# kamperh/segmentalist

Measured on AMD Instinct MI355X. Metric: Gibbs sweeps/sec (10k utts, D=100, K=1000) at 1/2/4/8 MI355X, higher is better.
Workload: dtype fp16 one-product filter + fp16x2 second stage, float32 reference arithmetic for the results; 1 GPU; SegmentalKMeansWordseg batch-synchronous sweep (BASELINE.json configs[2]); utterances=10000, landmarks_per_utt=20, n_slices_max=6, embeddings=1050000, D=100, K=1000, parallelism=utterance shards x1, ONE all-gather of the packed block statistics per sweep, collective=none (single process), sweep_launch=plain launches, corpus=one device holds all rows, device_memory_allocated_bytes_rank0=1237140480, components_after=815

## Files before the change

segmentalist_amd/csrc/segk_segment.hip:

```cpp
#include "segk_kmeans_dev.h"
#include "segk_segment_dev.h"


__global__ void k_kmeans_segment(segk_corpus c, segk_kmeans m, const int32_t *utts, int utt0, int n_utts,
                                 int n_min, int n_max, double wip, segk_cand cand, uint8_t *boundaries,
                                 int32_t *old_tok, int32_t *new_tok, int32_t *new_k, int32_t *n_old,
                                 int32_t *n_new, int32_t *n_flag, double *out_total, int32_t *status, int band_cap,
                                 int wave_bytes)
{
    extern __shared__ __attribute__((aligned(16))) char smem[];
    (void)n_min;
    const int lane = threadIdx.x & 63, wv = threadIdx.x >> 6;
    const int slot = blockIdx.x * (blockDim.x >> 6) + wv;
    if (slot >= n_utts) return;
    const int u = utts ? utts[slot] : utt0 + slot;
    const int N = c.lengths[u];
    const int W = (n_max > 0 && n_max < N) ? n_max : N;
    const int nb = N * W;
    const int64_t triMax = (int64_t)c.N_max * (c.N_max + 1) / 2;
    const int32_t *vid = c.vec_ids + (int64_t)u * triMax;
    const double *dur = c.durations + (int64_t)u * triMax;
    const bool band = c.band_ids != nullptr && c.band_W == W && W > 0;
    const int32_t *bandi = band ? c.band_ids + (int64_t)u * c.N_max * c.band_W : nullptr;
    const double *bandd = band ? c.band_dur + (int64_t)u * c.N_max * c.band_W : nullptr;
    uint8_t *gbnd = boundaries + (int64_t)u * c.N_max;

    char *base = smem + (size_t)wv * wave_bytes;
    double *bvec = (double *)base;
    double *gam = bvec + band_cap;
    int32_t *bk = (int32_t *)(gam + c.N_max + 1);
    int32_t *bid = bk + band_cap;
    int32_t *l_old = bid + band_cap;
    int32_t *l_new = l_old + c.N_max;
    int32_t *l_newk = l_new + c.N_max;
    int32_t *l_cnt = l_newk + c.N_max;
    uint8_t *l_bnd = (uint8_t *)(l_cnt + 2);

    for (int i = lane; i < nb; i += 64) {
        const int t = i / W + 1, w = i % W, s = t - 1 - w;
        int id = -1;
        double v = NEG_INF_D;
        int k = -1;
        if (s >= 0) {
            const int j = t * (t - 1) / 2 + s;
            id = band ? bandi[i] : vid[j];
            if (id >= 0) {
                k = cand.k[id];
                const double dd = band ? bandd[i] : dur[j];
                v = isnan(dd) ? NEG_INF_D : cand.s[id] * dd;
            }
        }
        bid[i] = id;
        bk[i] = k;
        bvec[i] = v + wip;
    }
    for (int j = lane; j < N; j += 64) l_bnd[j] = gbnd[j];
    WAVE_SYNC();
    if (lane == 0) {
#define V_(t, s) bvec[((t) - 1) * W + ((t) - 1 - (s))]
#define ID_(t, s) (((t) - 1 - (s)) < W ? bid[((t) - 1) * W + ((t) - 1 - (s))] : vid[(t) * ((t) - 1) / 2 + (s)])
        int no = 0, jp = 0;
        for (int j = 0; j < N; j++)
            if (l_bnd[j]) {
                int id = ID_(j + 1, jp);
                if (id >= 0) l_old[no++] = id;
                jp = j + 1;
            }
        gam[0] = 0.0;
        for (int t = 1; t < N; t++) {
            int lo = t - W < 0 ? 0 : t - W;
            double best = NEG_INF_D;
            for (int s = lo; s < t; s++) {
                double v = V_(t, s) + gam[s];
                if (v > best) best = v;
            }
            gam[t] = best;
        }
        for (int j = 0; j < N; j++) l_bnd[j] = 0;
        l_bnd[N - 1] = 1;
        int t = N;
        double total = 0.0;
        int lo = 0;
        for (;;) {
            lo = t - W < 0 ? 0 : t - W;
            bool all_inf = true;
            for (int s = lo; s < t; s++)
                if (V_(t, s) + gam[s] != NEG_INF_D) { all_inf = false; break; }
            if (all_inf) {
                while (all_inf) {
                    t = t - 1;
                    if (t == 0) break;
                    lo = t - W < 0 ? 0 : t - W;
                    all_inf = true;
                    for (int s = lo; s < t; s++)
                        if (V_(t, s) + gam[s] != NEG_INF_D) { all_inf = false; break; }
                }
                l_bnd[(t - 1 + N) % N] = 1;
            }
            int k = 1;
            if (t > 0) {
                double best = NEG_INF_D;
                bool first = true;
                for (int s = t - 1; s >= lo; s--) {
                    double v = V_(t, s) + gam[s];
                    if (first || v > best) { best = v; k = t - s; first = false; }
                }
                total += V_(t, t - k);
            } else {
                total += V_(N, N - 1);
            }
            if (t - k - 1 < 0) break;
            l_bnd[t - k - 1] = 1;
            t = t - k;
        }
        int nn = 0, bad = 0, nf = 0;
        const int Kact = *m.K;
        jp = 0;
        for (int j = 0; j < N; j++)
            if (l_bnd[j]) {
                int tt = j + 1, w = tt - 1 - jp;
                if (w >= W || bid[(tt - 1) * W + w] < 0) bad = 1;
                else {
                    l_new[nn] = bid[(tt - 1) * W + w];
                    l_newk[nn] = bk[(tt - 1) * W + w];
                    if (l_newk[nn] >= Kact) nf++;
                    nn++;
                }
                jp = j + 1;
            }
        out_total[u] = total;
        n_old[u] = no;
        n_new[u] = nn;
        if (n_flag) n_flag[u] = nf;
        l_cnt[0] = no;
        l_cnt[1] = nn;
        if (bad) atomicOr(status, 1);
#undef V_
#undef ID_
    }
    WAVE_SYNC();
    const int no = l_cnt[0], nn = l_cnt[1];
    for (int j = lane; j < N; j += 64) gbnd[j] = l_bnd[j];
    for (int j = lane; j < no; j += 64) old_tok[(int64_t)u * c.N_max + j] = l_old[j];
    for (int j = lane; j < c.N_max; j += 64) {
        if (j < nn) new_tok[(int64_t)u * c.N_max + j] = l_new[j];
        new_k[(int64_t)u * c.N_max + j] = j < nn ? l_newk[j] : -1;
    }
}

__global__ __launch_bounds__(256) void k_kmeans_segment_w8(segk_corpus c, segk_kmeans m, const int32_t *utts, int utt0, int n_utts,
                                    int n_max, double wip, segk_cand cand, uint8_t *boundaries, int32_t *old_tok,
                                    int32_t *new_tok, int32_t *new_k, int32_t *n_old, int32_t *n_new, int32_t *n_flag,
                                    double *out_total, int32_t *status, int band_cap, int wave_bytes)
{
    extern __shared__ __attribute__((aligned(16))) char smem[];
    const int lane = threadIdx.x & 63, wv = threadIdx.x >> 6;
    const int slot = blockIdx.x * (blockDim.x >> 6) + wv;
    SEGK_TSTAMP(0, 0);
    if (slot >= n_utts) return;
    const int u = utts ? utts[slot] : utt0 + slot;
    const int N = c.lengths[u];
    const int W = (n_max > 0 && n_max < N) ? n_max : N;
    const int64_t triMax = (int64_t)c.N_max * (c.N_max + 1) / 2;
    const int32_t *vid = c.vec_ids + (int64_t)u * triMax;
    const double *dur = c.durations + (int64_t)u * triMax;
    const bool band = c.band_ids != nullptr && c.band_W == W && W > 0;
    const int32_t *bandi = band ? c.band_ids + (int64_t)u * c.N_max * c.band_W : nullptr;
    const double *bandd = band ? c.band_dur + (int64_t)u * c.N_max * c.band_W : nullptr;
    uint8_t *gbnd = boundaries + (int64_t)u * c.N_max;

    char *base = smem + (size_t)wv * wave_bytes;
    double *bvec = (double *)base;
    double *gam = bvec + c.N_max * 8;
    int32_t *bk = (int32_t *)(gam + c.N_max + 12);
    int32_t *bid = bk + band_cap;
    int32_t *l_old = bid + band_cap;
    int32_t *l_new = l_old + c.N_max;
    int32_t *l_newk = l_new + c.N_max;
    int32_t *l_cnt = l_newk + c.N_max;

    {
        const int w = lane & 7;
        for (int z0 = 0; z0 < N; z0 += 32) {
            int id[4], kq[4];
            double dd[4], sc[4];
#pragma unroll
            for (int z = 0; z < 4; z++) {
                const int r = z0 + 8 * z + (lane >> 3), t = r + 1, sp = t - 1 - w;
                id[z] = -1;
                dd[z] = 0.0;
                if (r < N && w < W && sp >= 0) {
                    const int j = t * (t - 1) / 2 + sp;
                    id[z] = band ? bandi[r * W + w] : vid[j];
                    dd[z] = band ? bandd[r * W + w] : dur[j];
                }
            }
#pragma unroll
            for (int z = 0; z < 4; z++) {
                kq[z] = -1;
                sc[z] = 0.0;
                if (id[z] >= 0) {
                    kq[z] = cand.k[id[z]];
                    sc[z] = cand.s[id[z]];
                }
            }
#pragma unroll
            for (int z = 0; z < 4; z++) {
                const int r = z0 + 8 * z + (lane >> 3);
                if (r < N) {
                    double v = NEG_INF_D;
                    if (id[z] >= 0) v = isnan(dd[z]) ? NEG_INF_D : sc[z] * dd[z];
                    if (w < W) {
                        bid[r * W + w] = id[z];
                        bk[r * W + w] = kq[z];
                    }
                    bvec[r * 8 + w] = v + wip;
                }
            }
        }
    }
    const unsigned long long oldb = __ballot(lane < N && gbnd[lane < N ? lane : 0] != 0);
    WAVE_SYNC();
    SEGK_TSTAMP(0, 1);
    {
        const int no_ = seg_old_tokens_wave(bid, vid, N, W, oldb, l_old, lane);
        if (lane == 0) l_cnt[0] = no_;
    }
    double total;
    {
        unsigned long long newb_, keep_;
        int e_, k_, x_, f_;
        seg_w8_uniform(bvec, gam, bid, bk, N, W, *m.K, l_new, l_newk, l_cnt, &total, lane, newb_, keep_, e_, k_, x_, f_);
    }
    WAVE_SYNC();
    SEGK_TSTAMP(0, 2);
    if (lane == 0) {
        out_total[u] = total;
        n_old[u] = l_cnt[0];
        n_new[u] = l_cnt[1];
        if (n_flag) n_flag[u] = l_cnt[4];
        if (l_cnt[5]) atomicOr(status, 1);
    }
    WAVE_SYNC();
    const int no = l_cnt[0], nn = l_cnt[1];
    const unsigned long long newb = ((unsigned long long)(unsigned int)l_cnt[3] << 32) | (unsigned int)l_cnt[2];
    if (lane < N) gbnd[lane] = (uint8_t)((newb >> lane) & 1ull);
    for (int j = lane; j < no; j += 64) old_tok[(int64_t)u * c.N_max + j] = l_old[j];
    for (int j = lane; j < c.N_max; j += 64) {
        if (j < nn) new_tok[(int64_t)u * c.N_max + j] = l_new[j];
        new_k[(int64_t)u * c.N_max + j] = j < nn ? l_newk[j] : -1;
    }
    SEGK_TSTAMP_MAX(0, 3);
}

__device__ double dev_logsumexp(const double *a, int n)
{
    double mx = a[0], s = 0.0;
    for (int j = 1; j < n; j++)
        if (a[j] > mx) mx = a[j];
    for (int j = 0; j < n; j++) s += exp(a[j] - mx);
    return log(s) + mx;
}

__global__ void k_dp_tri(int kind, const double *vecs, const int32_t *Ns, const int64_t *offs, int n_prob,
                         int n_min, int n_max, double log_p_continue, double anneal_temp,
                         const double *uniforms, int64_t u_stride, uint8_t *bounds, int64_t b_stride,
                         double *totals, int32_t *n_draws, int32_t *status, double *work, int64_t w_stride)
{
    const int p = blockIdx.x * blockDim.x + threadIdx.x;
    if (p >= n_prob) return;
    const int N = Ns[p];
    const double *vec = vecs + offs[p];
    const int64_t L = (int64_t)N * (N + 1) / 2;
    uint8_t *bnd = bounds + p * b_stride;
    double *a = work + p * w_stride;
    double *w = a + N;
    double *pr = w + N + 1;
    const double *us = uniforms ? uniforms + p * u_stride : nullptr;
    for (int j = 0; j < N; j++) { a[j] = 1.0; bnd[j] = 0; }
    bnd[N - 1] = 1;
    a[0] = 0.0;
    int64_t i = 0;
    for (int t = 1; t < N; t++) {
        int lo = (n_max == 0 || t - n_max < 0) ? 0 : t - n_max;
        int n = t - lo;
        bool all_inf = true;
        double best = NEG_INF_D;
        for (int s = lo; s < t; s++) {
            double v = vec[i + s] + a[s];
            w[s - lo] = v;
            if (v != NEG_INF_D) all_inf = false;
            if (v > best) best = v;
        }
        if (kind == 2) a[t] = all_inf ? NEG_INF_D : dev_logsumexp(w, n) + log_p_continue;
        else a[t] = best;
        i += t;
    }
    int t = N, nd = 0, lo = 0;
    double total = 0.0;
    for (;;) {
        i = (int64_t)(t - 1) * t / 2;
        lo = (n_max == 0 || t - n_max < 0) ? 0 : t - n_max;
        bool all_inf = true;
        for (int s = lo; s < t; s++)
            if (vec[i + s] + a[s] != NEG_INF_D) { all_inf = false; break; }
        if (all_inf) {
            while (all_inf) {
                t = t - 1;
                if (t == 0) break;
                i = (int64_t)(t - 1) * t / 2;
                lo = (n_max == 0 || t - n_max < 0) ? 0 : t - n_max;
                all_inf = true;
                for (int s = lo; s < t; s++)
                    if (vec[i + s] + a[s] != NEG_INF_D) { all_inf = false; break; }
            }
            bnd[(t - 1 + N) % N] = 1;
        }
        int k = 1;
        int n = 1;
        if (t > 0) {
            n = t - lo;
            for (int s = lo; s < t; s++) w[s - lo] = vec[i + s] + a[s];
        } else {
            w[0] = NEG_INF_D;
        }
        if (kind == 0) {
            if (t > 0) {
                double best = NEG_INF_D;
                bool first = true;
                for (int s = t - 1; s >= lo; s--) {
                    double v = w[s - lo];
                    if (first || v > best) { best = v; k = t - s; first = false; }
                }
            }
        } else if (kind == 1) {
            if (t > 0) {
                double lse = dev_logsumexp(w, n);
                double best = 0.0;
                bool first = true;
                for (int s = t - 1; s >= lo; s--) {
                    double q = exp(w[s - lo] - lse);
                    if (first || q > best) { best = q; k = t - s; first = false; }
                }
            }
        } else {
            double lse = dev_logsumexp(w, n);
            if (anneal_temp != 1.0) {
                for (int j = 0; j < n; j++) pr[j] = w[n - 1 - j] - lse;
                double inv = 1. / anneal_temp;
                for (int j = 0; j < n; j++) w[j] = inv * pr[j];
                double lse2 = dev_logsumexp(w, n);
                for (int j = 0; j < n; j++) pr[j] = exp(w[j] - lse2);
            } else {
                for (int j = 0; j < n; j++) pr[j] = exp(w[n - 1 - j] - lse);
            }
            double uu = us[nd];
            nd++;
            int kk = n - 1;
            for (int j = 0; j < n; j++) {
                uu = uu - pr[j];
                if (uu < 0) { kk = j; break; }
            }
            k = kk + 1;
        }
        int64_t idx = i + t - k;
        if (idx < 0) idx += L;
        total += vec[idx];
        if (t - k - 1 < 0) break;
        bnd[t - k - 1] = 1;
        t = t - k;
    }
    totals[p] = total;
    if (n_draws) n_draws[p] = nd;
    if (status) status[p] = (kind == 2 && total == NEG_INF_D) ? 1 : 0;
}


extern "C" {

int32_t segk_kmeans_segment(segk_ctx *ctx, const segk_corpus *c, const segk_kmeans *m, const int32_t *utts,
                            int32_t utt0, int32_t n_utts, int32_t n_slices_min, int32_t n_slices_max, double wip,
                            const segk_cand *cand, uint8_t *boundaries, int32_t *old_tok, int32_t *new_tok,
                            int32_t *new_k, int32_t *n_old, int32_t *n_new, int32_t *n_flag, double *out_total,
                            int32_t *status, void *stream)
{
    int rc = check_corpus(c);
    if (rc) return rc;
    SEGK_REQUIRE(n_slices_min == 0 || n_slices_min == 1,
                 "n_slices_min must be 0 or 1 (>= 2 crashes in the reference, SURVEY 8(c))");
    SEGK_REQUIRE(n_slices_max >= 0, "n_slices_max");
    SEGK_REQUIRE(utts != nullptr || (utt0 >= 0 && utt0 + n_utts <= c->n_utt), "utterance range");
    if (n_utts <= 0) return SEGK_OK;
    hipStream_t st = (hipStream_t)stream;
    const int W = (n_slices_max > 0 && n_slices_max < c->N_max) ? n_slices_max : c->N_max;
    const int band_cap = c->N_max * W;
    size_t wave_bytes = (size_t)(band_cap + c->N_max + 1) * sizeof(double)
                        + (size_t)(2 * band_cap + 3 * c->N_max + 8) * sizeof(int32_t) + (size_t)c->N_max;
    wave_bytes = (wave_bytes + 15) & ~(size_t)15;
    size_t w8_bytes = (size_t)(c->N_max * 8 + c->N_max + 12) * sizeof(double)
                      + (size_t)(2 * band_cap + 3 * c->N_max + 8) * sizeof(int32_t) + (size_t)c->N_max;
    w8_bytes = (w8_bytes + 15) & ~(size_t)15;
    int waves = 4;
    while (waves > 1 && waves * wave_bytes > 64 * 1024) waves >>= 1;
    size_t lds = waves * wave_bytes;
    if (lds > 160 * 1024) {
        segk_set_error("segk_kmeans_segment: band of %d x %d spans needs %zu B of LDS (> 160 KiB); "
                       "set n_slices_max", c->N_max, W, lds);
        return SEGK_ERR_UNSUPPORTED;
    }
    if (lds > 48 * 1024)
        SEGK_CHECK_HIP(hipFuncSetAttribute((const void *)k_kmeans_segment, hipFuncAttributeMaxDynamicSharedMemorySize,
                                           (int)lds));
    (void)ctx;
    segk_tstamp_bind();
    if (n_slices_max >= 1 && n_slices_max <= 8 && c->N_max <= 64 && segk_env_int("SEGK_SEGMENT_GENERIC", 0) == 0) {
        int w8w = 4;
        while (w8w > 1 && w8w * w8_bytes > 64 * 1024) w8w >>= 1;
        hipLaunchKernelGGL(k_kmeans_segment_w8, dim3((n_utts + w8w - 1) / w8w), dim3(64 * w8w), w8w * w8_bytes, st, *c, *m, utts, utt0,
                           n_utts, n_slices_max, wip, *cand, boundaries, old_tok, new_tok, new_k, n_old, n_new, n_flag,
                           out_total, status, band_cap, (int)w8_bytes);
        SEGK_LAUNCH_CHECK();
        return SEGK_OK;
    }
    hipLaunchKernelGGL(k_kmeans_segment, dim3((n_utts + waves - 1) / waves), dim3(64 * waves), lds, st, *c, *m, utts,
                       utt0, n_utts, n_slices_min, n_slices_max, wip, *cand, boundaries, old_tok, new_tok, new_k, n_old,
                       n_new, n_flag, out_total, status, band_cap, (int)wave_bytes);
    SEGK_LAUNCH_CHECK();
    return SEGK_OK;
}

int32_t segk_dp_tri(segk_ctx *ctx, int32_t kind, const double *vecs, const int32_t *Ns, const int64_t *offs,
                    int32_t n_prob, int32_t n_slices_min, int32_t n_slices_max, double log_p_continue,
                    double anneal_temp, const double *uniforms, int64_t u_stride, uint8_t *bounds,
                    int64_t b_stride, double *totals, int32_t *n_draws, int32_t *status, double *work,
                    int64_t w_stride, void *stream)
{
    (void)ctx;
    SEGK_REQUIRE(kind >= 0 && kind <= 2, "kind");
    SEGK_REQUIRE(n_slices_min == 0 || n_slices_min == 1, "n_slices_min must be 0 or 1");
    SEGK_REQUIRE(kind != 2 || uniforms != nullptr, "uniforms required for forward_backward");
    if (n_prob <= 0) return SEGK_OK;
    hipLaunchKernelGGL(k_dp_tri, dim3((n_prob + 63) / 64), dim3(64), 0, (hipStream_t)stream, kind, vecs, Ns, offs,
                       n_prob, n_slices_min, n_slices_max, log_p_continue, anneal_temp, uniforms, u_stride, bounds,
                       b_stride, totals, n_draws, status, work, w_stride);
    SEGK_LAUNCH_CHECK();
    return SEGK_OK;
}

}
```

segmentalist_amd/csrc/segk_segment_dev.h:

```cpp
#pragma once
#include "segk_kmeans_dev.h"

#define WAVE_SYNC()                                             \
    do {                                                        \
        __builtin_amdgcn_fence(__ATOMIC_ACQ_REL, "wavefront");  \
        __builtin_amdgcn_wave_barrier();                        \
    } while (0)


__device__ __forceinline__ int seg_old_tokens_wave(const int32_t *bid, const int32_t *vid, int N, int W, unsigned long long oldb,
                                                   int32_t *l_old, int lane)
{
    const bool bit = lane < N && ((oldb >> lane) & 1ull);
    const unsigned long long below = oldb & ((1ull << lane) - 1ull);
    const int jp = below ? 64 - __clzll((long long)below) : 0;
    int id = -1;
    if (bit) {
        const int t = lane + 1, w = lane - jp;
        id = w < W ? bid[(t - 1) * W + w] : vid[t * (t - 1) / 2 + jp];
    }
    const unsigned long long keep = __ballot(bit && id >= 0);
    if (bit && id >= 0) l_old[__popcll(keep & ((1ull << lane) - 1ull))] = id;
    return __popcll(keep);
}

__device__ __forceinline__ double seg_readlane_f64(double v, int l)
{
    const int lo = __builtin_amdgcn_readlane(__double2loint(v), l), hi = __builtin_amdgcn_readlane(__double2hiint(v), l);
    return __hiloint2double(hi, lo);
}
template <int WW>
__device__ __forceinline__ void seg_forward_uniform(const double *bvec8, double *gamp, int N, int lane)
{
    double ring[8];
#pragma unroll
    for (int s = 0; s < 8; s++) ring[s] = NEG_INF_D;
    ring[0] = 0.0;
    double va[WW], vb[WW];
    auto fetch = [&](double (&dst)[WW], int row) {
        const double2 *src = reinterpret_cast<const double2 *>(bvec8 + (size_t)row * 8);
#pragma unroll
        for (int h = 0; h < WW / 2; h++) {
            const double2 d = src[h];
            dst[2 * h] = d.x;
            dst[2 * h + 1] = d.y;
        }
    };
    fetch(va, 0);
    for (int t0 = 1; t0 <= N; t0 += 8) {
#pragma unroll
        for (int half = 0; half < 2; half++) {
            if (half == 1 && t0 + 4 > N) break;
#pragma unroll
            for (int jj = 0; jj < 4; jj++) {
                const int j = 4 * half + jj;
                const int t = t0 + j;
                double (&v)[WW] = (j & 1) ? vb : va;
                fetch((j & 1) ? va : vb, t < N ? t : N - 1);
                double x[WW];
#pragma unroll
                for (int w = 0; w < WW; w++) x[w] = v[w] + ring[(j - w) & 7];
#pragma unroll
                for (int h = 1; h < WW; h <<= 1)
#pragma unroll
                    for (int w = 0; w + h < WW; w += 2 * h) x[w] = fmax(x[w], x[w + h]);
                ring[(j + 1) & 7] = x[0];
                if (lane == 0) gamp[8 + t] = x[0];
            }
        }
    }
}
__device__ __forceinline__ void seg_w8_uniform(const double *bvec8, double *gamp, const int32_t *bid, const int32_t *bk, int N, int W,
                                               int Kact, int32_t *l_new, int32_t *l_newk, int32_t *l_cnt, double *total_out, int lane,
                                               unsigned long long &newb_out, unsigned long long &keep_out, int &id_out, int &k_out,
                                               int &entry_out, int &n_flag_out, unsigned long long *tstamp = nullptr)
{
#define SEG_U_STAMP(i) do { if (tstamp && lane == 0) tstamp[i] = wall_clock64(); } while (0)
    N = __builtin_amdgcn_readfirstlane(N);
    W = __builtin_amdgcn_readfirstlane(W);
    SEG_U_STAMP(0);
    if (lane < 8) gamp[lane] = NEG_INF_D;
    if (lane == 0) gamp[8] = 0.0;
    if (W <= 2) seg_forward_uniform<2>(bvec8, gamp, N, lane);
    else if (W <= 4) seg_forward_uniform<4>(bvec8, gamp, N, lane);
    else if (W <= 6) seg_forward_uniform<6>(bvec8, gamp, N, lane);
    else seg_forward_uniform<8>(bvec8, gamp, N, lane);
    WAVE_SYNC();
    SEG_U_STAMP(1);
    int kbv = 0;
    double cv = 0.0;
    if (lane < N) {
        const double mx = gamp[8 + lane + 1];
        double v[8], g[8];
        const double2 *src = reinterpret_cast<const double2 *>(bvec8 + (size_t)lane * 8);
#pragma unroll
        for (int h = 0; h < 4; h++) {
            const double2 d = src[h];
            v[2 * h] = d.x;
            v[2 * h + 1] = d.y;
        }
#pragma unroll
        for (int w = 0; w < 8; w++) g[w] = gamp[8 + lane - w];
        if (mx != NEG_INF_D) {
#pragma unroll
            for (int w = 7; w >= 0; w--)
                if (v[w] + g[w] == mx) {
                    kbv = w + 1;
                    cv = v[w];
                }
        }
    }
    SEG_U_STAMP(2);
    unsigned long long newb = 1ull << (N - 1);
    int t = N;
    double total = 0.0;
    bool blocked = false;
    for (;;) {
        const int kb = __builtin_amdgcn_readlane(kbv, t - 1);
        if (kb == 0) {
            blocked = true;
            break;
        }
        total += seg_readlane_f64(cv, t - 1);
        t = t - kb;
        if (t < 1) break;
        newb |= 1ull << (t - 1);
    }
    if (blocked)
        for (;;) {
            int kb = __builtin_amdgcn_readlane(kbv, t - 1);
            if (kb == 0) {
                do {
                    t = t - 1;
                    if (t == 0) break;
                    kb = __builtin_amdgcn_readlane(kbv, t - 1);
                } while (kb == 0);
                if (t == 0) {
                    newb |= 1ull << (N - 1);
                    total += bvec8[(size_t)(N - 1) * 8];
                    break;
                }
                newb |= 1ull << (t - 1);
            }
            total += seg_readlane_f64(cv, t - 1);
            t = t - kb;
            if (t < 1) break;
            newb |= 1ull << (t - 1);
        }
    SEG_U_STAMP(3);
    {
        const bool bit = lane < N && ((newb >> lane) & 1ull);
        const unsigned long long below = newb & ((1ull << lane) - 1ull);
        const int jp = below ? 64 - __clzll((long long)below) : 0;
        const int w = lane - jp;
        int id = -1, kk = -1;
        if (bit && w < W) {
            id = bid[lane * W + w];
            kk = bk[lane * W + w];
        }
        const bool valid = bit && id >= 0;
        const unsigned long long keep = __ballot(valid), badm = __ballot(bit && !valid), fl = __ballot(valid && kk >= Kact);
        if (valid) {
            const int r = __popcll(keep & ((1ull << lane) - 1ull));
            l_new[r] = id;
            l_newk[r] = kk;
        }
        if (lane == 0) {
            l_cnt[1] = __popcll(keep);
            l_cnt[2] = (int32_t)(newb & 0xffffffffull);
            l_cnt[3] = (int32_t)(newb >> 32);
            l_cnt[4] = __popcll(fl);
            l_cnt[5] = badm != 0ull;
        }
        newb_out = newb;
        keep_out = keep;
        id_out = valid ? id : -1;
        k_out = kk;
        entry_out = lane * W + (w < W ? w : 0);
        n_flag_out = __popcll(fl);
    }
    *total_out = total;
    SEG_U_STAMP(4);
#undef SEG_U_STAMP
}
```

Baseline: 6840 sweeps/s.

## Pack two utterances per wavefront in segmentation kernel when N_max <= 32

Adds a w8x2 variant of the banded segmentation kernel that splits each 64-lane wavefront into two 32-lane halves, each processing its own utterance. The forward DP, traceback walk and token extraction are reworked to use per-half ballots and lane offsets. With landmarks_per_utt=20, a full wave previously left most lanes idle, so this aims to double lane utilization and halve the number of waves launched. The cost is more LDS per wave, serialized tracebacks for both halves within one wave, and the forward pass running to the longer of the two lengths.

```diff
diff --git a/segmentalist_amd/csrc/segk_segment.hip b/segmentalist_amd/csrc/segk_segment.hip
--- a/segmentalist_amd/csrc/segk_segment.hip
+++ b/segmentalist_amd/csrc/segk_segment.hip
@@ -249,6 +249,112 @@
     for (int j = lane; j < c.N_max; j += 64) {
         if (j < nn) new_tok[(int64_t)u * c.N_max + j] = l_new[j];
         new_k[(int64_t)u * c.N_max + j] = j < nn ? l_newk[j] : -1;
+    }
+    SEGK_TSTAMP_MAX(0, 3);
+}
+
+__global__ __launch_bounds__(256, 7) void k_kmeans_segment_w8x2(segk_corpus c, segk_kmeans m, const int32_t *utts, int utt0, int n_utts,
+                                    int n_max, double wip, segk_cand cand, uint8_t *boundaries, int32_t *old_tok,
+                                    int32_t *new_tok, int32_t *new_k, int32_t *n_old, int32_t *n_new, int32_t *n_flag,
+                                    double *out_total, int32_t *status, int band_cap, int wave_bytes)
+{
+    extern __shared__ __attribute__((aligned(16))) char smem[];
+    const int lane = threadIdx.x & 63, wv = threadIdx.x >> 6, h = lane >> 5, hl = lane & 31;
+    const int first = 2 * (blockIdx.x * (blockDim.x >> 6) + wv);
+    SEGK_TSTAMP(0, 0);
+    if (first >= n_utts) return;
+    const bool live = first + h < n_utts;
+    const int slot = live ? first + h : first;
+    const int u = utts ? utts[slot] : utt0 + slot;
+    const int N = c.lengths[u];
+    const int W = (n_max > 0 && n_max < N) ? n_max : N;
+    const int64_t triMax = (int64_t)c.N_max * (c.N_max + 1) / 2;
+    const int32_t *vid = c.vec_ids + (int64_t)u * triMax;
+    const double *dur = c.durations + (int64_t)u * triMax;
+    const bool band = c.band_ids != nullptr && c.band_W == W && W > 0;
+    const int32_t *bandi = band ? c.band_ids + (int64_t)u * c.N_max * c.band_W : nullptr;
+    const double *bandd = band ? c.band_dur + (int64_t)u * c.N_max * c.band_W : nullptr;
+    uint8_t *gbnd = boundaries + (int64_t)u * c.N_max;
+    const int Nm = max(__builtin_amdgcn_readlane(N, 0), __builtin_amdgcn_readlane(N, 32));
+
+    char *base_w = smem + (size_t)wv * 2 * wave_bytes;
+    char *base = base_w + (size_t)h * wave_bytes;
+    double *bvec = (double *)base;
+    double *gam = bvec + c.N_max * 8;
+    int32_t *bk = (int32_t *)(gam + c.N_max + 12);
+    int32_t *bid = bk + band_cap;
+    int32_t *l_old = bid + band_cap;
+    int32_t *l_new = l_old + c.N_max;
+    int32_t *l_newk = l_new + c.N_max;
+    int32_t *l_cnt = l_newk + c.N_max;
+
+    {
+        const int w = hl & 7;
+        for (int z0 = 0; z0 < Nm; z0 += 16) {
+            int id[4], kq[4];
+            double dd[4], sc[4];
+#pragma unroll
+            for (int z = 0; z < 4; z++) {
+                const int r = z0 + 4 * z + (hl >> 3), t = r + 1, sp = t - 1 - w;
+                id[z] = -1;
+                dd[z] = 0.0;
+                if (r < N && w < W && sp >= 0) {
+                    const int j = t * (t - 1) / 2 + sp;
+                    id[z] = band ? bandi[r * W + w] : vid[j];
+                    dd[z] = band ? bandd[r * W + w] : dur[j];
+                }
+            }
+#pragma unroll
+            for (int z = 0; z < 4; z++) {
+                kq[z] = -1;
+                sc[z] = 0.0;
+                if (id[z] >= 0) {
+                    kq[z] = cand.k[id[z]];
+                    sc[z] = cand.s[id[z]];
+                }
+            }
+#pragma unroll
+            for (int z = 0; z < 4; z++) {
+                const int r = z0 + 4 * z + (hl >> 3);
+                if (r < Nm) {
+                    double v = NEG_INF_D;
+                    if (id[z] >= 0) v = isnan(dd[z]) ? NEG_INF_D : sc[z] * dd[z];
+                    if (r < N && w < W) {
+                        bid[r * W + w] = id[z];
+                        bk[r * W + w] = kq[z];
+                    }
+                    bvec[r * 8 + w] = v + wip;
+                }
+            }
+        }
+    }
+    const unsigned int oldb = (unsigned int)(__ballot(hl < N && gbnd[hl < N ? hl : 0] != 0) >> (32 * h));
+    WAVE_SYNC();
+    SEGK_TSTAMP(0, 1);
+    {
+        const int no_ = seg_old_tokens_half(bid, vid, N, W, oldb, l_old, hl, h);
+        if (hl == 0) l_cnt[0] = no_;
+    }
+    double total;
+    seg_w8_uniform_x2(bvec, gam, bid, bk, N, W, *m.K, l_new, l_newk, l_cnt, &total, hl, h, (const double *)base_w, wave_bytes / 8);
+    WAVE_SYNC();
+    SEGK_TSTAMP(0, 2);
+    if (hl == 0 && live) {
+        out_total[u] = total;
+        n_old[u] = l_cnt[0];
+        n_new[u] = l_cnt[1];
+        if (n_flag) n_flag[u] = l_cnt[4];
+        if (l_cnt[5]) atomicOr(status, 1);
+    }
+    WAVE_SYNC();
+    if (!live) return;
+    const int no = l_cnt[0], nn = l_cnt[1];
+    const unsigned int newb = (unsigned int)l_cnt[2];
+    if (hl < N) gbnd[hl] = (uint8_t)((newb >> hl) & 1u);
+    if (hl < no) old_tok[(int64_t)u * c.N_max + hl] = l_old[hl];
+    if (hl < c.N_max) {
+        if (hl < nn) new_tok[(int64_t)u * c.N_max + hl] = l_new[hl];
+        new_k[(int64_t)u * c.N_max + hl] = hl < nn ? l_newk[hl] : -1;
     }
     SEGK_TSTAMP_MAX(0, 3);
 }
@@ -415,6 +521,15 @@
     segk_tstamp_bind();
     if (n_slices_max >= 1 && n_slices_max <= 8 && c->N_max <= 64 && segk_env_int("SEGK_SEGMENT_GENERIC", 0) == 0) {
         int w8w = 4;
+        if (c->N_max <= 32) {
+            while (w8w > 1 && w8w * 2 * w8_bytes > 64 * 1024) w8w >>= 1;
+            const int n_waves = (n_utts + 1) / 2;
+            hipLaunchKernelGGL(k_kmeans_segment_w8x2, dim3((n_waves + w8w - 1) / w8w), dim3(64 * w8w), w8w * 2 * w8_bytes, st, *c, *m,
+                               utts, utt0, n_utts, n_slices_max, wip, *cand, boundaries, old_tok, new_tok, new_k, n_old, n_new, n_flag,
+                               out_total, status, band_cap, (int)w8_bytes);
+            SEGK_LAUNCH_CHECK();
+            return SEGK_OK;
+        }
         while (w8w > 1 && w8w * w8_bytes > 64 * 1024) w8w >>= 1;
         hipLaunchKernelGGL(k_kmeans_segment_w8, dim3((n_utts + w8w - 1) / w8w), dim3(64 * w8w), w8w * w8_bytes, st, *c, *m, utts, utt0,
                            n_utts, n_slices_max, wip, *cand, boundaries, old_tok, new_tok, new_k, n_old, n_new, n_flag,
diff --git a/segmentalist_amd/csrc/segk_segment_dev.h b/segmentalist_amd/csrc/segk_segment_dev.h
--- a/segmentalist_amd/csrc/segk_segment_dev.h
+++ b/segmentalist_amd/csrc/segk_segment_dev.h
@@ -183,3 +183,131 @@
     SEG_U_STAMP(4);
 #undef SEG_U_STAMP
 }
+
+__device__ __forceinline__ int seg_old_tokens_half(const int32_t *bid, const int32_t *vid, int N, int W, unsigned int oldb,
+                                                   int32_t *l_old, int hl, int h)
+{
+    const bool bit = hl < N && ((oldb >> hl) & 1u);
+    const unsigned int below = oldb & ((1u << hl) - 1u);
+    const int jp = below ? 32 - __clz((int)below) : 0;
+    int id = -1;
+    if (bit) {
+        const int t = hl + 1, w = hl - jp;
+        id = w < W ? bid[(t - 1) * W + w] : vid[t * (t - 1) / 2 + jp];
+    }
+    const unsigned int keep = (unsigned int)(__ballot(bit && id >= 0) >> (32 * h));
+    if (bit && id >= 0) l_old[__popc(keep & ((1u << hl) - 1u))] = id;
+    return __popc(keep);
+}
+__device__ __forceinline__ void seg_walk_half(int kbv, double cv, int N, int l0, const double *bvec8, unsigned int &newb_out,
+                                              double &total_out)
+{
+    unsigned int newb = 1u << (N - 1);
+    int t = N;
+    double total = 0.0;
+    bool blocked = false;
+    for (;;) {
+        const int kb = __builtin_amdgcn_readlane(kbv, l0 + t - 1);
+        if (kb == 0) {
+            blocked = true;
+            break;
+        }
+        total += seg_readlane_f64(cv, l0 + t - 1);
+        t = t - kb;
+        if (t < 1) break;
+        newb |= 1u << (t - 1);
+    }
+    if (blocked)
+        for (;;) {
+            int kb = __builtin_amdgcn_readlane(kbv, l0 + t - 1);
+            if (kb == 0) {
+                do {
+                    t = t - 1;
+                    if (t == 0) break;
+                    kb = __builtin_amdgcn_readlane(kbv, l0 + t - 1);
+                } while (kb == 0);
+                if (t == 0) {
+                    newb |= 1u << (N - 1);
+                    total += bvec8[(size_t)(N - 1) * 8];
+                    break;
+                }
+                newb |= 1u << (t - 1);
+            }
+            total += seg_readlane_f64(cv, l0 + t - 1);
+            t = t - kb;
+            if (t < 1) break;
+            newb |= 1u << (t - 1);
+        }
+    newb_out = newb;
+    total_out = total;
+}
+__device__ __forceinline__ void seg_w8_uniform_x2(const double *bvec8, double *gamp, const int32_t *bid, const int32_t *bk, int N, int W,
+                                                  int Kact, int32_t *l_new, int32_t *l_newk, int32_t *l_cnt, double *total_out, int hl,
+                                                  int h, const double *bvec8_w, int half_doubles)
+{
+    const int N0 = __builtin_amdgcn_readlane(N, 0), N1 = __builtin_amdgcn_readlane(N, 32);
+    const int W0 = __builtin_amdgcn_readlane(W, 0), W1 = __builtin_amdgcn_readlane(W, 32);
+    const int Nm = N0 > N1 ? N0 : N1, Wm = W0 > W1 ? W0 : W1;
+    if (hl < 8) gamp[hl] = NEG_INF_D;
+    if (hl == 0) gamp[8] = 0.0;
+    if (Wm <= 2) seg_forward_uniform<2>(bvec8, gamp, Nm, hl);
+    else if (Wm <= 4) seg_forward_uniform<4>(bvec8, gamp, Nm, hl);
+    else if (Wm <= 6) seg_forward_uniform<6>(bvec8, gamp, Nm, hl);
+    else seg_forward_uniform<8>(bvec8, gamp, Nm, hl);
+    WAVE_SYNC();
+    int kbv = 0;
+    double cv = 0.0;
+    if (hl < N) {
+        const double mx = gamp[8 + hl + 1];
+        double v[8], g[8];
+        const double2 *src = reinterpret_cast<const double2 *>(bvec8 + (size_t)hl * 8);
+#pragma unroll
+        for (int q = 0; q < 4; q++) {
+            const double2 d = src[q];
+            v[2 * q] = d.x;
+            v[2 * q + 1] = d.y;
+        }
+#pragma unroll
+        for (int w = 0; w < 8; w++) g[w] = gamp[8 + hl - w];
+        if (mx != NEG_INF_D) {
+#pragma unroll
+            for (int w = 7; w >= 0; w--)
+                if (v[w] + g[w] == mx) {
+                    kbv = w + 1;
+                    cv = v[w];
+                }
+        }
+    }
+    unsigned int nb0, nb1;
+    double tt0, tt1;
+    seg_walk_half(kbv, cv, N0, 0, bvec8_w, nb0, tt0);
+    seg_walk_half(kbv, cv, N1, 32, bvec8_w + half_doubles, nb1, tt1);
+    const unsigned int newb = h ? nb1 : nb0;
+    {
+        const bool bit = hl < N && ((newb >> hl) & 1u);
+        const unsigned int below = newb & ((1u << hl) - 1u);
+        const int jp = below ? 32 - __clz((int)below) : 0;
+        const int w = hl - jp;
+        int id = -1, kk = -1;
+        if (bit && w < W) {
+            id = bid[hl * W + w];
+            kk = bk[hl * W + w];
+        }
+        const bool valid = bit && id >= 0;
+        const unsigned int keep = (unsigned int)(__ballot(valid) >> (32 * h)), badm = (unsigned int)(__ballot(bit && !valid) >> (32 * h)),
+                           fl = (unsigned int)(__ballot(valid && kk >= Kact) >> (32 * h));
+        if (valid) {
+            const int r = __popc(keep & ((1u << hl) - 1u));
+            l_new[r] = id;
+            l_newk[r] = kk;
+        }
+        if (hl == 0) {
+            l_cnt[1] = __popc(keep);
+            l_cnt[2] = (int32_t)newb;
+            l_cnt[3] = 0;
+            l_cnt[4] = __popc(fl);
+            l_cnt[5] = badm != 0u;
+        }
+    }
+    *total_out = h ? tt1 : tt0;
+}
```

After: 7008 sweeps/s (median of 6 runs). +2.5%, better.
